# usra-riacs/Nonlocal-Monte-Carlo

Hardware: AMD Instinct MI355X
Metric: spin-updates/s (replicas x spins x sweeps / s), NPT sweep + swap rounds, schedule construction included (higher is better)
Workload: dtype f64 field + 53-bit uniform (the reference's arithmetic, NMC/nmc.py:86-87; on this +-J instance the fp64 field is an exact integer and the fp64 acceptance test an exact integer threshold per field value: bit-identical to the sweep-by-sweep fp64 kernel and the fp64 oracle); 1 GPU; NPT heat-bath sweeps + replica exchange, sparse +-J spin glass (C4 per GPU); spins=10000, edges=30000, replicas_per_gpu=256, replicas_total=256, sweeps_per_round=10, swap_pairs_per_round=77, rng=philox4x32-10, order=one permutation per sweep, plan_chunk_rounds=256

## Files before the change

nonlocal-monte-carlo_amd/csrc/nlmc.hip:

```cpp
#include "../../include/nlmc.h"
#include "nlmc_kernels.h"
#include "nlmc_pt_icm.h"
#include "nlmc_apt.h"
#include "nlmc_lbp.h"
#include "nlmc_nmc.h"
#include "nlmc_probe.h"
#include "nlmc_big.h"
#include "nlmc_host.h"

#include <dlfcn.h>

#include <algorithm>
#include <chrono>
#include <thread>
#include <climits>
#include <cmath>
#include <cstdio>
#include <cstdlib>
#include <cstring>
#include <string>
#include <vector>

namespace {

// ... 256 lines not shown
{
    const size_t i = 3 * t;
    const uint8_t kind = t < c->ev_kind.size() ? c->ev_kind[t] : 0;
    lev = sw = 0.f;
    HIP_TRY(c, hipEventSynchronize(c->events[i + 2]));
    if (kind == 0) {
        HIP_TRY(c, hipEventElapsedTime(&lev, c->events[i], c->events[i + 1]));
        HIP_TRY(c, hipEventElapsedTime(&sw, c->events[i + 1], c->events[i + 2]));
    } else if (kind == 1) {
        HIP_TRY(c, hipEventElapsedTime(&sw, c->events[i], c->events[i + 2]));
    } else {
        HIP_TRY(c, hipEventElapsedTime(&lev, c->events[i], c->events[i + 2]));
    }
    return NLMC_OK;
}

int sweep_block(int n)
{
    if (const char *s = getenv("NLMC_SWEEP_NT")) {
        int v = atoi(s);
        if (v >= 64 && v <= 1024 && v % 64 == 0) return v;
    }
    int nt = ((n + 7) / 8 + 63) / 64 * 64;
    return std::min(1024, std::max(64, nt));
}

int sweep_block_for(int n, bool f64_philox, bool f32_diag = false)
{
    return std::min(f64_philox ? 512 : f32_diag ? 768 : 1024, sweep_block(n));
}

int ensure_lds(nlmc_ctx *c, int slot, const void *func, size_t bytes)
{
    if (bytes > (size_t)158 * 1024) return fail(c, NLMC_ERR_UNSUPPORTED, "instance too large for the LDS-resident kernels of this build");
    if (bytes <= (size_t)60 * 1024 || bytes <= c->lds_opt[slot]) return NLMC_OK;
    HIP_TRY(c, hipFuncSetAttribute(func, hipFuncAttributeMaxDynamicSharedMemorySize, (int)bytes));
    c->lds_opt[slot] = bytes;
    return NLMC_OK;
}

int level_block(int n)
{
    int nt = ((n + 3) / 4 + 63) / 64 * 64;
    return std::min(1024, std::max(64, nt));
}

void launch_energy(nlmc_ctx *c, unsigned count, hipStream_t st, const EnergyArgs &a)
{
    const dim3 nt(c->n >= 4096 ? 1024 : 256);
    if (c->big) hipLaunchKernelGGL(k_energy<true>, dim3(count), nt, 0, st, a);
    else hipLaunchKernelGGL(k_energy<false>, dim3(count), nt, (size_t)c->n_pad, st, a);
}

int launch_energy_self(nlmc_ctx *c, double *dev_out)
{
    EnergyArgs a{};
    a.g = c->g;
    a.spins = c->spins.p;
    a.stride = c->n_pad;
    a.out = dev_out;
    a.efix = c->efix.p;
    a.escale = c->escale;
    if (c->n_chains > 0) launch_energy(c, (unsigned)c->n_chains, c->stream, a);
    HIP_TRY(c, hipGetLastError());
    return NLMC_OK;
}

int run_levelize(nlmc_ctx *c, int n_orders, const uint32_t *keys_in, int per_chain, int n_sweeps, uint32_t sweep0,
                 uint64_t seed, nlmc_ctx::Sched &sc, int ell_mode)
{
    if (n_orders <= 0) return NLMC_OK;
    if (ell_mode < 0) {
        BigLevelizeArgs b{};
        b.g = c->g;
        b.n_orders = n_orders;
        b.keys_in = keys_in;
        b.seed_lo = (uint32_t)seed; b.seed_hi = (uint32_t)(seed >> 32); b.sweep0 = sweep0;
        b.per_chain = per_chain; b.n_sweeps = n_sweeps; b.chain_base = c->chain_base;
        b.key = sc.bkey.p; b.lvl = sc.blvl.p; b.cur = sc.bcur.p;
        b.ord2 = sc.order.p; b.lvl_off = sc.lvl_off.p; b.nlev = sc.nlev.p; b.hi_max = sc.hi_max.p;
        HIP_TRY(c, c->big_flag.reserve(NLMC_BIG_PASSES));
        b.flag = c->big_flag.p;
        const unsigned gx = (unsigned)((c->n + 255) / 256);
        for (int ob = 0; ob < n_orders; ob += 65535) {
            const int no = std::min(65535, n_orders - ob);
            BigLevelizeArgs q = b;
            const size_t n = (size_t)c->n;
            q.n_orders = no;
            if (q.keys_in) q.keys_in += (size_t)ob * n;
            q.key = b.key ? b.key + (size_t)ob * n : nullptr; q.lvl += (size_t)ob * n; q.cur += (size_t)ob * (n + 2);
            q.ord2 += (size_t)ob * n; q.lvl_off += (size_t)ob * (n + 1); q.nlev += ob; q.hi_max += ob;
            if (!q.keys_in && per_chain && n_orders > 65535) return fail(c, NLMC_ERR_UNSUPPORTED, "more than 65535 per-chain orders of a long chain in one window");
            if (!q.keys_in) q.sweep0 = sweep0 + (uint32_t)ob;
            hipLaunchKernelGGL(k_blv_init, dim3(gx, no), dim3(256), 0, c->cur, q);
            HIP_TRY(c, hipGetLastError());
            bool settled = false;
            for (long long done = 0; !settled && done <= (long long)c->n + NLMC_BIG_PASSES; done += NLMC_BIG_PASSES) {
                int32_t fl[NLMC_BIG_PASSES];
                HIP_TRY(c, hipMemsetAsync(q.flag, 0, sizeof(fl), c->cur));
                for (int p = 0; p < NLMC_BIG_PASSES; ++p) hipLaunchKernelGGL(k_blv_pass, dim3(gx, no), dim3(256), 0, c->cur, q, p);
                HIP_TRY(c, hipGetLastError());
                HIP_TRY(c, hipMemcpyAsync(fl, q.flag, sizeof(fl), hipMemcpyDeviceToHost, c->cur));
                HIP_TRY(c, hipStreamSynchronize(c->cur));
                for (int p = 0; p < NLMC_BIG_PASSES; ++p) settled = settled || fl[p] == 0;
            }
            if (!settled) return fail(c, NLMC_ERR_STATE, "level schedule of a long chain did not settle");
            const unsigned gt = (unsigned)((c->n + NLMC_BIG_TILE - 1) / NLMC_BIG_TILE);
            hipLaunchKernelGGL(k_blv_hist, dim3(gt, no), dim3(256), 0, c->cur, q);
            hipLaunchKernelGGL(k_blv_scan, dim3(no), dim3(1024), 0, c->cur, q);
            hipLaunchKernelGGL(k_blv_place, dim3(gt, no), dim3(256), 0, c->cur, q);
            HIP_TRY(c, hipGetLastError());
        }
        return NLMC_OK;
    }
    LevelizeArgs a{};
    a.g = c->g;
    a.n_orders = n_orders;
    a.keys_in = keys_in;
    a.seed_lo = (uint32_t)seed;
    a.seed_hi = (uint32_t)(seed >> 32);
    a.sweep0 = sweep0;
    a.per_chain = per_chain;
    a.n_sweeps = n_sweeps;
    a.chain_base = c->chain_base;
    a.level_cap = sweep_block_for(c->n, ell_mode == 2, ell_mode == 1 && c->has_diag);
    a.ord2 = sc.order.p;
    a.lvl_off = sc.lvl_off.p;
    a.nlev = sc.nlev.p;
    a.hi_max = sc.hi_max.p;
    if (ell_mode == 1) { a.ell32 = sc.ell32.p; a.head32 = sc.head32.p; }
    if (ell_mode == 2) { a.ellc64 = sc.ellc64.p; a.ellv64 = sc.ellv64.p; a.headh64 = sc.headh64.p; a.pack16 = c->f64_pack16 ? 1 : 0; }
    const size_t lds_one = (size_t)(c->n + 2) * 4 + (((size_t)c->n * 2 + 3) / 4) * 4;
    const size_t lds_two = lds_one + (size_t)(c->n + 2) * 4;
    a.two_sided = lds_two + 16 <= (size_t)150 * 1024;
    const size_t lds = (a.two_sided ? lds_two : lds_one) + 16;
    { int rc = ensure_lds(c, 0, reinterpret_cast<const void *>(k_levelize), lds); if (rc) return rc; }
    hipLaunchKernelGGL(k_levelize, dim3(n_orders), dim3(level_block(c->n)), lds, c->cur, a);
    HIP_TRY(c, hipGetLastError());
    return NLMC_OK;
}

int fused_block(int n)
{
    if (getenv("NLMC_SWEEP_NT")) return std::max(256, sweep_block(n));
    const int nt = ((3 * n + 15) / 16 + 63) / 64 * 64;
    return std::min(1024, std::max(256, nt));
}

int fused_workers(int nt)
{
    const int waves = nt / 64;
    if (waves < 16) return waves - 1;
    if (const char *s = getenv("NLMC_FUSED_WORKERS")) { const int v = atoi(s); if (v >= 8 && v <= 16) return v; }
    return 15;
}

struct FusedLds { int neg_off, flags_off, u_off, u_bytes, snap_off, red_off, kt_off; size_t total; };
FusedLds fused_lds(int n, int n_pad, bool has_flags, bool with_out, bool with_neg, int kt_entries = 0)
{
    (void)n;
    FusedLds L{};
    L.neg_off = with_neg ? n_pad + 16 : 0;
    L.flags_off = (n_pad + 16) * (with_neg ? 2 : 1);
    int cur = L.flags_off + (has_flags ? n_pad + 16 : 0);
    cur = (cur + 15) / 16 * 16;
    L.u_off = cur;
    L.u_bytes = n_pad * 4;
    cur += 3 * L.u_bytes;
    L.snap_off = cur;
    if (with_out) cur += 3 * n_pad + 16;
    L.red_off = cur;
    L.kt_off = cur + 32;
    L.total = (size_t)cur + 32 + (size_t)kt_entries * 8;
    return L;
}

bool fused_addr_format(const nlmc_ctx *c)
{
    return c->sign8 && 2 * (c->n_pad + 16) <= 0xFFFF && fused_lds(c->n, c->n_pad, true, false, true).total <= (size_t)150 * 1024;
}

int fused_pstride(int n, int n_long, int T) { return (int)((((size_t)T * ((size_t)n + n_long) + 63) / 64 + NLMC_LCAP) * 64); }

int fused_gen0(int nt)
{
    const int waves = nt / 64;
    if (const char *s = getenv("NLMC_FUSED_GEN0")) { const int v = atoi(s); if (v >= 0 && v < waves) return v; }
    return waves / 2;
}

bool fused_supported(const nlmc_ctx *c, int T)
{
    if (getenv("NLMC_NO_FUSED") || c->big) return false;
    if (c->n < 256 || c->n > NLMC_FZ_SPT * 1024 || c->max_deg > 0x3FFF || T < 3 || T > NLMC_FUSED_TMAX) return false;
    if ((size_t)T * ((size_t)c->n + c->n_long) > ((size_t)1 << 22)) return false;
    if (c->n_pad + 16 > 0x3FFF) return false;
    (void)T;
    const FusedLds L = fused_lds(c->n, c->n_pad, true, false, false);
    if (3 * L.u_bytes / 4 > 0xFFFF) return false;
    return L.total <= (size_t)150 * 1024;
}

bool fused_f64_supported(const nlmc_ctx *c, int T)
{
    if (!c->f64_exact || c->xmax > 4095 || getenv("NLMC_NO_FUSED64")) return false;
    if (!fused_supported(c, T)) return false;
    return fused_lds(c->n, c->n_pad, false, false, fused_addr_format(c), 2 * c->xmax + 1).total <= (size_t)156 * 1024;
}

const void *fused_kernel(bool diag, bool flags, bool outs, int fmt, bool f64 = false)
{
    if (f64) {
#define NLMC_K64(D, O) {reinterpret_cast<const void *>(k_sweep_fused<D, false, O, NLMC_FMT_WIDE, true>), reinterpret_cast<const void *>(k_sweep_fused<D, false, O, NLMC_FMT_COMPACT, true>), \
                        reinterpret_cast<const void *>(k_sweep_fused<D, false, O, NLMC_FMT_ADDR, true>)}
        static const void *const t64[2][2][3] = {{NLMC_K64(false, false), NLMC_K64(false, true)}, {NLMC_K64(true, false), NLMC_K64(true, true)}};
#undef NLMC_K64
        return flags ? nullptr : t64[diag][outs][fmt];
    }
#define NLMC_K(D, F, O) {reinterpret_cast<const void *>(k_sweep_fused<D, F, O, NLMC_FMT_WIDE>), reinterpret_cast<const void *>(k_sweep_fused<D, F, O, NLMC_FMT_COMPACT>), \
                         reinterpret_cast<const void *>(k_sweep_fused<D, F, O, NLMC_FMT_ADDR>)}
    static const void *const table[2][2][2][3] = {{{NLMC_K(false, false, false), NLMC_K(false, false, true)}, {NLMC_K(false, true, false), NLMC_K(false, true, true)}},
                                                  {{NLMC_K(true, false, false), NLMC_K(true, false, true)}, {NLMC_K(true, true, false), NLMC_K(true, true, true)}}};
#undef NLMC_K
    static_assert(NLMC_FMT_WIDE == 0 && NLMC_FMT_COMPACT == 1 && NLMC_FMT_ADDR == 2, "table order");
    return table[diag][flags][outs][fmt];
}

struct SweepOut {
    int record_stride;
    int8_t *out_spins;
    double *out_energy;
    double *out_min_energy;
    int32_t *out_argmin;
    int8_t *out_argmin_state;
};

int run_fused(nlmc_ctx *c, int slot, int w, uint32_t sweep0, uint64_t seed, const double *tab_dev, int tab_cs, int tab_ss, bool use_slots,
              bool outs, bool want_energy, bool want_min, bool want_state, int rec, int t0, int n_total, bool f64 = false,
              const DeferSwap *defer = nullptr, double *sink_override = nullptr)
{
    const nlmc_ctx::FusedPlan &P = c->fz[slot];
    const int R = c->sub_count(), n = c->n, T = P.T;
    const size_t PS = (size_t)P.pstride;
    const int kt = f64 ? 2 * c->xmax + 1 : 0;
    const bool snap_lds = outs && fused_lds(c->n, c->n_pad, c->has_flags, true, P.fmt == NLMC_FMT_ADDR, kt).total <= (size_t)150 * 1024;
    const FusedLds L = fused_lds(c->n, c->n_pad, c->has_flags, snap_lds, P.fmt == NLMC_FMT_ADDR, kt);
    if (outs && !snap_lds) HIP_TRY(c, c->snap_g.reserve((size_t)R * (3 * (size_t)c->n_pad + 16)));
    const int variant = (outs ? 4 : 0) + (c->has_diag ? 2 : 0) + (c->has_flags ? 1 : 0);
    const void *kfun = fused_kernel(c->has_diag, c->has_flags, outs, P.fmt, f64);
    int lds_slot = f64 ? 48 + ((c->has_diag ? 2 : 0) + (outs ? 1 : 0)) * 3 + P.fmt : 24 + variant * 3 + P.fmt;
    if (defer) {
#define NLMC_KD(D, F64_) {reinterpret_cast<const void *>(k_sweep_fused<D, false, false, NLMC_FMT_WIDE, F64_, true>), reinterpret_cast<const void *>(k_sweep_fused<D, false, false, NLMC_FMT_COMPACT, F64_, true>), \
                          reinterpret_cast<const void *>(k_sweep_fused<D, false, false, NLMC_FMT_ADDR, F64_, true>)}
        static const void *const dtable[2][2][3] = {{NLMC_KD(false, false), NLMC_KD(false, true)}, {NLMC_KD(true, false), NLMC_KD(true, true)}};
#undef NLMC_KD
        kfun = (c->has_flags || outs) ? nullptr : dtable[c->has_diag][f64][P.fmt];
        lds_slot = 72 + ((c->has_diag ? 2 : 0) + (f64 ? 1 : 0)) * 3 + P.fmt;
    }
    if (!kfun) return fail(c, NLMC_ERR_STATE, "run_fused: no kernel for this combination (fp64 mode or deferred swap with phase flags / outputs)");
    { int rc = ensure_lds(c, lds_slot, kfun, L.total); if (rc) return rc; }
    const bool timed = c->ev_accumulate && (c->ev_every <= 1 || c->launches_total % c->ev_every == 0);
    hipEvent_t e0 = nullptr, e2 = nullptr;
    if (timed) {
        e0 = next_event(c);
        hipEvent_t e1 = next_event(c);
        e2 = next_event(c);
        if (!e0 || !e1 || !e2) return fail(c, NLMC_ERR_HIP, "hipEventCreate failed");
        tag_triple(c, 1);
        HIP_TRY(c, hipEventRecord(e0, c->cur));
    }
    SweepArgs a{};
    a.g = c->g;
    a.chain_base = c->chain_base;
    a.chain_list = c->sub_list();
    a.spins = c->spins.p;
    a.flags = c->has_flags ? c->flags.p : nullptr;
    a.temp_x = c->temp_x;
    a.lvl_off = P.loff.p + (size_t)w * (NLMC_LCAP + 1);
    a.nlev = P.nlev.p + w;
    a.hi_max = P.himax.p + w;
    a.ell32 = P.ell.p + (size_t)w * PS * NLMC_FZ_W;
    a.head32 = P.head.p + (size_t)w * PS;
    a.fsend = P.send.p + (size_t)w * T;
    a.fz_pstride = P.pstride;
    a.fz_fmt = P.fmt;
    if (w + 1 < P.windows && P.nlev_host[(size_t)w + 1] > 0 && !c->knob_no_warm) {
        a.warm_head = P.head.p + (size_t)(w + 1) * PS;
        a.warm_ell = P.ell.p + (size_t)(w + 1) * PS * NLMC_FZ_W;
        a.fz_npos_next = P.npos_host[(size_t)w + 1];
    }
    a.f_workers = P.workers;
    a.f_gen0 = P.gen0;
    a.f_gen_prio = c->knob_no_prio ? 0 : 1;
#ifdef NLMC_DEBUG_KNOBS
    a.dbg_flags = c->knob_dbg_flags;
#endif
    a.n_sweeps = T;
    a.sweep0 = sweep0;
    a.seed_lo = (uint32_t)seed; a.seed_hi = (uint32_t)(seed >> 32);
    a.tab = tab_dev; a.tab_cs = tab_cs; a.tab_ss = tab_ss;
    a.slot_of_chain = use_slots ? c->slot_of_chain.p : nullptr;
    a.efix = c->efix.p;
    a.energy_sink = sink_override ? sink_override : c->energy_sink;
    if (defer) a.defer = *defer;
    a.escale = c->escale;
    a.eshift = c->escale - c->qs;
    a.qinv = std::ldexp(1.0f, -c->qs);
// ... 2431 lines not shown
```

nonlocal-monte-carlo_amd/csrc/nlmc_kernels.h:

```cpp
#pragma once
#include "nlmc_device.h"

struct EdgeQ { int32_t col; int32_t q; };

struct CsrDev {
    int n, n_pad;
    const int32_t *rowptr;
    const int32_t *col;
    const double *val64;
    const EdgeQ *edge32;
    const double *h64;
    const int32_t *hq;
};

struct LevelizeArgs {
    CsrDev g;
    int n_orders;
    const uint32_t *keys_in;
    uint32_t seed_lo, seed_hi, sweep0;
    int per_chain;
    int n_sweeps;
    int chain_base;
    int level_cap;
    int two_sided;
// ... 1294 lines not shown
                const int l = l0 + (tid & 63);
                const unsigned long long m = __ballot((l < nl) && (loff[l + 1] - loff[l] > 64));
                if (m) n_bar = l0 + 64 - __clzll((long long)m);
            }
            const bool role_long = (Pf<T, PK>::W > 8) && ((tid & ~63) < a.hi_max[oid]);
            if (role_long) run_levels<T, DIAG, true, false, NoGen, PK>(a, x, ur, loff, so, nl, n_bar, cb0, cb1, esc);
            else run_levels<T, DIAG, false, false, NoGen, PK>(a, x, ur, loff, so, nl, n_bar, cb0, cb1, esc);

            if (dbuf && t + 1 < a.n_sweeps) {
                const int oid_n = a.per_chain ? (x.ob * a.n_sweeps + t + 1) : (t + 1);
                const int nl_n = a.nlev[oid_n];
                const bool wave0_busy = n_bar < nl;
                if (nl_n < NLMC_LCAP && (!wave0_busy || nt > 64)) {
                    const int hid = wave0_busy ? tid - 64 : tid, hcnt = wave0_busy ? nt - 64 : nt;
                    if (hid >= 0) {
                        T *ur_n = reinterpret_cast<T *>(reinterpret_cast<unsigned char *>(ur0) + (size_t)(pb ^ 1) * a.lds_u_stride);
                        int *loff_n = reinterpret_cast<int *>(reinterpret_cast<unsigned char *>(loff0) + (size_t)(pb ^ 1) * a.lds_loff_stride);
                        const int32_t *__restrict__ off_n = a.lvl_off + (size_t)oid_n * (n + 1);
                        fill_uniforms(ur_n, n, tt + 1u, gc, a.seed_lo, a.seed_hi, hid, hcnt);
                        for (int l = hid; l <= nl_n; l += hcnt) loff_n[l] = off_n[l];
                    }
                    prefilled = true;
                }
            }
        } else {
            for (int l = 0; l < nl; ++l) {
                const int lo = off[l], hi = off[l + 1];
                for (int i = lo + tid; i < hi; i += nt) {
                    Pf<T, PK> pe;
                    typename Pf<T, PK>::View vw;
                    vw.bind(a, so, n);
                    pe.template issue<true>(vw, i, true);
                    update_spin<T, DIAG, true, false, PK>(a, x, ur, pe, so, i, cb0, cb1, esc);
                }
                __syncthreads();
            }
        }
#ifdef NLMC_STAMPS
        const long long e0 = (long long)__builtin_readcyclecounter();
#endif
        __syncthreads();
        sweep_epilogue(a, x, t);
#ifdef NLMC_STAMPS
        st_epi += (long long)__builtin_readcyclecounter() - e0;
#endif
    }
#ifdef NLMC_STAMPS
    if (a.dbg && (tid & 63) == 0) {
        long long *d = a.dbg + ((size_t)c * 16 + (tid >> 6)) * 8;
        d[0] = st_u[0]; d[1] = st_u[1]; d[2] = st_u[2]; d[3] = st_u[3]; d[4] = st_u[4]; d[5] = st_fill;
        d[6] = (long long)__builtin_readcyclecounter() - st_begin; d[7] = st_epi;
    }
#endif
    chain_store(a, x);
}

template <int FMT> struct FusedItem {
    static constexpr int NE = NLMC_FZ_W;
    static constexpr int NP = FMT == NLMC_FMT_WIDE ? NE / 2 : FMT == NLMC_FMT_COMPACT ? NE / 4 : NE / 8;
    nlmc_i2 hd;
    nlmc_i4 pk[NP];
    __device__ __forceinline__ int word(int i) const { const int p = i >> 2, j = i & 3; return j == 0 ? pk[p].x : j == 1 ? pk[p].y : j == 2 ? pk[p].z : pk[p].w; }
    __device__ __forceinline__ unsigned col(int q) const
    {
        if (FMT == NLMC_FMT_WIDE) return (unsigned)word(2 * q);
        if (FMT == NLMC_FMT_COMPACT) return (unsigned)word(q) >> 16;
        return (q & 1) ? (unsigned)word(q >> 1) >> 16 : (unsigned)word(q >> 1) & 0xFFFFu;
    }
    __device__ __forceinline__ int val(int q) const
    {
        if (FMT == NLMC_FMT_WIDE) return word(2 * q + 1);
        return (int)(short)(word(q) & 0xFFFF);
    }
};

__device__ __forceinline__ float4 thresholds4(const u32x4 &r)
{
    float4 v;
    v.x = threshold_spec(r.x);
    v.y = threshold_spec(r.y);
    v.z = threshold_spec(r.z);
    v.w = threshold_spec(r.w);
    return v;
}

struct FusedGenParams { uint32_t gc; int gtid, gnt, nblk, nj, Tn; };
struct FusedWin {
    const int32_t *lvl_off;
    const int32_t *fsend;
    const EdgeQ *ell;
    const int2 *head;
    const int2 *warm_head;
    const EdgeQ *warm_ell;
    int npos_next;
    int nl, hi_max;
    uint32_t sweep0;
};
#ifdef NLMC_DEBUG_KNOBS
#define NLMC_GEN_DBG_OFF_COND (a.dbg_flags & 1)
#define NLMC_GEN_DBG_PHILOX if (a.dbg_flags & 8) g_r = u32x4{(uint32_t)b * 2654435761u, (uint32_t)b ^ gp.gc, (uint32_t)g_u * 40503u + (uint32_t)b, ~(uint32_t)b}; else
#define NLMC_GEN_DBG_LOGIT if (a.dbg_flags & 16) dst[b] = nlmc_f4{__uint_as_float(g_r.x & 0x3FFFFFFFu), __uint_as_float(g_r.y & 0x3FFFFFFFu), __uint_as_float(g_r.z & 0x3FFFFFFFu), __uint_as_float(g_r.w & 0x3FFFFFFFu)}; else
#else
#define NLMC_GEN_DBG_OFF_COND false
#define NLMC_GEN_DBG_PHILOX
#define NLMC_GEN_DBG_LOGIT
#endif
#define NLMC_GEN_STATE int g_u = 2, g_slot = 2, g_w0 = 0, g_wend = 0, g_wlen = 1, g_acc = 0, g_sidx = 0; u32x4 g_r{0u, 0u, 0u, 0u}; \
    const uint32_t g_seed_lo = a.seed_lo, g_seed_hi = a.seed_hi, g_sweep0 = W.sweep0; const int g_u_off = a.lds_u_off, g_u_stride = a.lds_u_stride; \
    const int32_t *const g_fsend = W.fsend;
#define NLMC_GEN_NSTEP (g_f64 ? 2 : 3)
#define NLMC_GEN_ARM(a, gp)                                                                                             \
    {                                                                                                                   \
        typedef const int32_t __attribute__((address_space(4))) *const_i32_;                                            \
        g_sidx = 0; g_acc = 0;                                                                                          \
        if (g_u < gp.Tn) {                                                                                              \
            const const_i32_ send_ = (const_i32_)(uintptr_t)g_fsend;                                                    \
            g_w0 = g_u >= 3 ? __builtin_amdgcn_readfirstlane(send_[g_u - 3]) : -1;                                      \
            g_wend = __builtin_amdgcn_readfirstlane(send_[g_u - 2]);                                                    \
            g_wlen = max(1, g_wend - g_w0);                 \
        } else g_w0 = 0x7FFFFFFF;                                                                                       \
    }
#define NLMC_GEN_STEP(a, gp)                                                                                            \
    {                                                                                                                   \
        const int call_ = g_sidx / NLMC_GEN_NSTEP, ph_ = g_sidx - call_ * NLMC_GEN_NSTEP;                               \
        const int b = gp.gtid + call_ * gp.gnt;                                                                         \
        if (ph_ == 0) {                                                                                                 \
            NLMC_GEN_DBG_PHILOX                                                                                         \
            g_r = philox4x32_rounds(u32x4{(uint32_t)b, g_sweep0 + (uint32_t)g_u, gp.gc, NLMC_TAG_UNIFORM}, g_seed_lo, g_seed_hi, 0, 5); \
        } else if (g_f64) {                                                                                             \
            typedef nlmc_i4 __attribute__((address_space(3))) *lds_i4_;                                                 \
            g_r = philox4x32_rounds(g_r, g_seed_lo, g_seed_hi, 5, 5);                                                   \
            if (b < gp.nblk) ((lds_i4_)(uintptr_t)(unsigned)(g_u_off + g_slot * g_u_stride))[b] = nlmc_i4{(int)(g_r.x >> 5), (int)(g_r.y >> 5), (int)(g_r.z >> 5), (int)(g_r.w >> 5)}; \
        } else if (ph_ == 1) {                                                                                          \
            NLMC_GEN_DBG_PHILOX                                                                                         \
            g_r = philox4x32_rounds(g_r, g_seed_lo, g_seed_hi, 5, 5);                                                   \
        } else if (b < gp.nblk) {                                                                                       \
            typedef nlmc_f4 __attribute__((address_space(3))) *lds_f4_;             \
            const lds_f4_ dst = (lds_f4_)(uintptr_t)(unsigned)(g_u_off + g_slot * g_u_stride);                  \
            NLMC_GEN_DBG_LOGIT                                                                                          \
            { const float4 t4 = thresholds4(g_r); dst[b] = nlmc_f4{t4.x, t4.y, t4.z, t4.w}; }                           \
        }                                                                                                               \
        ++g_sidx;                                                                                                       \
    }
#define NLMC_GEN(a, gp, l)                                                                                              \
    if (!(NLMC_GEN_DBG_OFF_COND) && (l) > g_w0) {                                                                       \
        g_acc += NLMC_GEN_NSTEP * gp.nj;                                                                                \
        while (g_acc >= g_wlen) { g_acc -= g_wlen; if (g_sidx < NLMC_GEN_NSTEP * gp.nj) NLMC_GEN_STEP(a, gp) }          \
        if (__builtin_expect((l) == g_wend, 0)) {                                                                       \
            while (g_sidx < NLMC_GEN_NSTEP * gp.nj) NLMC_GEN_STEP(a, gp)                                                \
            ++g_u; g_slot = g_slot == 2 ? 0 : g_slot + 1; NLMC_GEN_ARM(a, gp)                                           \
        }                                                                                                               \
    }

template <bool DIAG, bool FLAGS, bool PAIR, bool GEN, int FMT, bool OUT = false, bool F64 = false>
__device__ __forceinline__ void fused_levels(const SweepArgs &a, const FusedWin &W, unsigned char *lds_raw, int wv, int lane, int nl, float cq0,
                                             float cq1, long long &e_loc, const FusedGenParams gp)
{
    constexpr bool g_f64 = F64;
    static_assert(!(F64 && FLAGS), "fused fp64 windows: plain chains only (a scaled row's field is not an exact integer)");
    NLMC_GEN_STATE
    NLMC_GEN_ARM(a, gp)
    typedef const int32_t __attribute__((address_space(4))) *const_i32o;
    typedef const double __attribute__((address_space(4))) *const_f64o;
    const int o_npad = a.g.n_pad, o_b = blockIdx.x, o_c = a.chain_list ? a.chain_list[o_b] : o_b, o_tid = wv * 64 + lane;
    int o_t = 0, o_end = 0;
    unsigned o_lo = 0u;
    long long e_new = 0, E_run = 0, E_min = 0;
    int a_min = 0;
    float cqo0 = cq0, cqo1 = cq1, cqn0 = cq0, cqn1 = cq1;
    const int o_row = a.slot_of_chain ? a.slot_of_chain[a.chain_base + o_c] : o_c;
    int8_t *const snapg = (OUT && a.snap_g) ? a.snap_g + (size_t)o_b * (3 * (size_t)o_npad + 16) : nullptr;
#define NLMC_OCQ(t, j) ((float)((const_f64o)(uintptr_t)a.tab)[(size_t)o_row * a.tab_cs + (size_t)min((t), a.n_sweeps - 1) * a.tab_ss + (j)] * a.qinv)
    if (OUT) {
        o_end = ((const_i32o)(uintptr_t)W.fsend)[0];
        E_run = uniform64(a.efix[o_c]);
        E_min = a.emin ? uniform64(a.emin[o_c]) : 0x7FFFFFFFFFFFFFFFll;
        a_min = a.emin ? __builtin_amdgcn_readfirstlane(a.argmin[o_c]) : 0;
        cqn0 = NLMC_OCQ(1, 0); cqn1 = NLMC_OCQ(1, 1);
    }
    typedef FusedItem<FMT> Item;
    unsigned v_u_off = (unsigned)a.lds_u_off, v_neg_off = (unsigned)a.lds_neg_off;
    int v_eshift = a.eshift;
    asm volatile("" : "+v"(v_u_off), "+v"(v_neg_off), "+v"(v_eshift));
    unsigned v_kt0 = (unsigned)(a.lds_kt_off + 4 * a.f64_xmax), v_tie = a.f64_tie_mask;
    if (F64) asm volatile("" : "+v"(v_kt0), "+v"(v_tie));
    typedef const unsigned __attribute__((address_space(3))) *lds_u32;
    constexpr int NP = Item::NP, NE = Item::NE;
    const int plane_bytes = a.fz_pstride * 16;
    const __amdgpu_buffer_rsrc_t r_ell = __builtin_amdgcn_make_buffer_rsrc(const_cast<EdgeQ *>(W.ell), 0, (NLMC_FZ_W / 2) * plane_bytes, 0x00020000);
    const __amdgpu_buffer_rsrc_t r_head = __builtin_amdgcn_make_buffer_rsrc(const_cast<int2 *>(W.head), 0, a.fz_pstride * 8, 0x00020000);
    typedef const int32_t __attribute__((address_space(4))) *const_i32;
    const const_i32 loffp = (const_i32)(uintptr_t)W.lvl_off;
    auto lo = [&](int i) __attribute__((always_inline)) { return loffp[min(i, nl)]; };
    const int lane16 = lane * 16, oob = 0x7FF00000;
    typedef const int8_t __attribute__((address_space(3))) *lds_i8;
    typedef int8_t __attribute__((address_space(3))) *lds_i8w;
    typedef const uint8_t __attribute__((address_space(3))) *lds_u8;
    typedef const float __attribute__((address_space(3))) *lds_f32;

    auto issue = [&](Item &it, int c, bool has) __attribute__((always_inline)) {
#ifdef NLMC_DEBUG_KNOBS
        if (a.dbg_flags & 32) return;
#endif
        const int v16 = has ? lane16 : oob;
        it.hd = __builtin_amdgcn_raw_buffer_load_b64(r_head, v16 >> 1, c * 512, 0);
#pragma unroll
        for (int q = 0; q < NP; ++q) it.pk[q] = __builtin_amdgcn_raw_buffer_load_b128(r_ell, v16, c * 1024 + q * plane_bytes, 0);
    };
    auto update = [&](const Item &it, int lv) __attribute__((always_inline)) {
        (void)lv;
#ifdef NLMC_DEBUG_KNOBS
        if (a.dbg_flags & 2) { asm volatile("" :: "v"(it.hd.x), "v"(it.pk[0].x), "v"(it.pk[Item::NP - 1].x)); return; }
#endif
        const int hx = it.hd.x;
#ifdef NLMC_DEBUG_KNOBS
        const unsigned ka = (a.dbg_flags & 1024) ? (unsigned)((lane & 31) * 4 + (lane >> 5)) : (unsigned)hx & 0x3FFFu;
        const float wk = *(lds_f32)(uintptr_t)(((a.dbg_flags & 1024) ? (unsigned)(lane * 4) : (((unsigned)hx >> 16) << 2)) + (unsigned)a.lds_u_off);
#else
        const unsigned ka = (unsigned)hx & 0x3FFFu;
        const float wk = *(lds_f32)(uintptr_t)((((unsigned)hx >> 16) << 2) + v_u_off);
#endif
        int so = (int)*(lds_i8)(uintptr_t)ka;
        unsigned f = 0u;
        if (FLAGS) f = (unsigned)*(lds_u8)(uintptr_t)(ka + (unsigned)a.lds_flags_off);
        int sj[NE];
#ifdef NLMC_DEBUG_KNOBS
        if (a.dbg_flags & 512) {
#pragma unroll
            for (int q = 0; q < NE; ++q) sj[q] = (int)*(lds_i8)(uintptr_t)(unsigned)((lane & 31) * 4 + q * 132 + (lane >> 5));
        } else
#endif
        {
#pragma unroll
            for (int q = 0; q < NE; ++q) sj[q] = (int)*(lds_i8)(uintptr_t)it.col(q);
        }
        asm volatile("" : "+v"(so));
        int X0 = it.hd.y, X1 = 0, Xd = 0;
#pragma unroll
        for (int q = 0; q < NE; q += 2) {
            if (FMT == NLMC_FMT_ADDR) {
                X0 += sj[q];
                X1 += sj[q + 1];
            } else {
                X0 += __mul24(it.val(q), sj[q]);
                X1 += __mul24(it.val(q + 1), sj[q + 1]);
            }
        }
        if (DIAG) {
#pragma unroll
            for (int q = 0; q < NE; ++q) {
                if (FMT == NLMC_FMT_ADDR) Xd += (it.col(q) == ka || it.col(q) == ka + v_neg_off) ? sj[q] : 0;
                else Xd += (it.col(q) == ka) ? __mul24(it.val(q), sj[q]) : 0;
            }
        }
        int X = X0 + X1;
        bool second = false;
        if (PAIR) {
            if (__builtin_amdgcn_ballot_w64((hx & 0x4000) != 0) != 0ull) {
                if (hx & 0x4000) {
                    const int rs = a.g.rowptr[ka], re = a.g.rowptr[ka + 1];
#pragma clang loop vectorize(disable) unroll(disable)
                    for (int e = rs + 2 * NLMC_FZ_W; e < re; ++e) {
                        const EdgeQ t = a.g.edge32[e];
                        const int pr = __mul24(t.q, (int)*(lds_i8)(uintptr_t)(unsigned)t.col);
                        X += pr;
                        if (DIAG && (unsigned)t.col == ka) Xd += pr;
                    }
                }
            }
            const bool pair = (hx & 0x8000) != 0;
            const int Xp = __builtin_amdgcn_mov_dpp(X, 0xB1, 0xF, 0xF, true);
            X += pair ? Xp : 0;
            if (DIAG) { const int Xdp = __builtin_amdgcn_mov_dpp(Xd, 0xB1, 0xF, 0xF, true); Xd += pair ? Xdp : 0; }
            second = pair && (lane & 1);
        }
        bool up64 = false;
        if (F64) {
            const unsigned hk = __float_as_uint(wk);
            const unsigned kaddr = ((unsigned)X << 2) + v_kt0;
#ifdef NLMC_DEBUG_KNOBS
            const unsigned kh = (a.dbg_flags & 16384) ? (unsigned)(X * 3000000 + 0x4000000) : *(lds_u32)(uintptr_t)kaddr;
#else
            const unsigned kh = *(lds_u32)(uintptr_t)kaddr;
#endif
            up64 = hk < kh;
            const bool tie = ((hk ^ kh) & v_tie) == 0u;
            if (__builtin_expect(__builtin_amdgcn_ballot_w64(tie) != 0ull, 0)) {
                if (tie) {
                    typedef const int32_t __attribute__((address_space(4))) *const_i32s;
                    const unsigned tw_ = (unsigned)hx >> 16, np_ = (unsigned)a.g.n_pad;
                    int t_ = tw_ >= 3u * np_ ? 3 : tw_ >= 2u * np_ ? 2 : tw_ >= np_ ? 1 : 0;
                    while (t_ + 3 < a.n_sweeps && lv > ((const_i32s)(uintptr_t)W.fsend)[t_]) t_ += 3;
                    const u32x4 r_ = philox4x32_10(ka >> 2, W.sweep0 + (uint32_t)t_, gp.gc, NLMC_TAG_UNIFORM_LO, a.seed_lo, a.seed_hi);
                    const unsigned lw_ = (ka & 2u) ? ((ka & 1u) ? r_.w : r_.z) : ((ka & 1u) ? r_.y : r_.x);
                    const unsigned lo_ = lw_ >> 6;
                    const unsigned kl = *(lds_u32)(uintptr_t)(kaddr + 4u * (unsigned)(2 * a.f64_xmax + 1));
                    up64 = hk < kh || (hk == kh && lo_ < kl);
                }
            }
        }
        if (!OUT) {
            const float z = ((FLAGS && f == 1u) ? cq1 : cq0) * (float)X;
            int sn = F64 ? (up64 ? 1 : -1) : (z < wk) ? 1 : -1;
            if (FLAGS) sn = (f >= 2u) ? so : sn;
            const int cv = (PAIR && second) ? 0 : (so - sn) << v_eshift;
            e_loc += (long long)(DIAG ? X - Xd : X) * (long long)cv;
            *(lds_i8w)(uintptr_t)ka = (int8_t)sn;
            if (FMT == NLMC_FMT_ADDR) *(lds_i8w)(uintptr_t)(ka + v_neg_off) = (int8_t)-sn;
        } else {
            const unsigned tw = (unsigned)hx >> 16;
            const bool is_old = tw - o_lo < (unsigned)o_npad;
            const float cqa = is_old ? cqo0 : cqn0, cqb = is_old ? cqo1 : cqn1;
            const float z = ((FLAGS && f == 1u) ? cqb : cqa) * (float)X;
            int sn = F64 ? (up64 ? 1 : -1) : (z < wk) ? 1 : -1;
            if (FLAGS) sn = (f >= 2u) ? so : sn;
            const int cv = (PAIR && second) ? 0 : (so - sn) << v_eshift, cvo = is_old ? cv : 0;
            const long long Xt = (long long)(DIAG ? X - Xd : X);
            e_loc += Xt * (long long)cvo;
            e_new += Xt * (long long)(cv - cvo);
            *(lds_i8w)(uintptr_t)ka = (int8_t)sn;
            if (FMT == NLMC_FMT_ADDR) *(lds_i8w)(uintptr_t)(ka + v_neg_off) = (int8_t)-sn;
            if (snapg) snapg[tw] = (int8_t)sn;
            else *(lds_i8w)(uintptr_t)(tw + (unsigned)a.lds_snap_off) = (int8_t)sn;
        }
    };
#define NLMC_OUT_PRE                                                                                                    \
    {                                                                                                                   \
        if (snapg) asm volatile("s_waitcnt vmcnt(0)" ::: "memory");            \
        const long long w_ = wave_sum_i64(e_loc);                                                                       \
        long long *red_ = reinterpret_cast<long long *>(lds_raw + a.lds_red_off);                                       \
        if (lane == 0 && w_ != 0) atomicAdd(reinterpret_cast<unsigned long long *>(&red_[o_t % 3]), (unsigned long long)w_); \
    }
#define NLMC_OUT_POST                                                                                                   \
    {                                                                                                                   \
        long long *red_ = reinterpret_cast<long long *>(lds_raw + a.lds_red_off);                                       \
        const int slot_ = o_t % 3, tg_ = a.t0 + o_t;                                                                    \
        E_run += uniform64(red_[slot_]);                                                                                \
        const bool better_ = a.emin && E_run < E_min && (tg_ % a.min_stride == 0);    \
        if (better_) { E_min = E_run; a_min = tg_; }                                                                    \
        if (o_tid == 0) {                                                                                               \
            red_[(o_t + 2) % 3] = 0;                                \
            if (a.etrace) a.etrace[(size_t)o_b * a.trace_sweeps + tg_] = E_run;                                         \
        }                                                                                                               \
        const unsigned char *snap_ = snapg ? reinterpret_cast<const unsigned char *>(snapg) + (size_t)slot_ * o_npad              \
                                           : lds_raw + a.lds_snap_off + (size_t)slot_ * o_npad;                         \
        if (better_ && a.best) {                                                                                        \
            int4 *dst_ = reinterpret_cast<int4 *>(a.best + (size_t)o_c * o_npad);                                       \
            const int4 *src_ = reinterpret_cast<const int4 *>(snap_);                                                   \
            if (snapg) for (int i_ = o_tid; i_ < o_npad / 16; i_ += a.f_workers * 64)                                  \
                reinterpret_cast<nlmc_i4 *>(dst_)[i_] = __builtin_nontemporal_load(&reinterpret_cast<const nlmc_i4 *>(src_)[i_]);   \
            else for (int i_ = o_tid; i_ < o_npad / 16; i_ += a.f_workers * 64) dst_[i_] = src_[i_];                    \
        }                                                                                                               \
        if (a.strace && tg_ % a.rec_stride == 0) {                                 \
            const int n_rec_ = (a.trace_sweeps + a.rec_stride - 1) / a.rec_stride;                                      \
            int8_t *dst_ = a.strace + ((size_t)o_b * n_rec_ + (size_t)(tg_ / a.rec_stride)) * a.g.n;                   \
            if (snapg) for (int i_ = o_tid; i_ < a.g.n; i_ += a.f_workers * 64) dst_[i_] = (int8_t)__builtin_nontemporal_load(&snap_[i_]); \
            else for (int i_ = o_tid; i_ < a.g.n; i_ += a.f_workers * 64) dst_[i_] = (int8_t)snap_[i_];                 \
        }                                                                                                               \
        e_loc = e_new; e_new = 0;                                                                                       \
        ++o_t;                                                                                                          \
        o_lo = (unsigned)((o_t % 3) * o_npad);                                                                          \
        o_end = o_t < a.n_sweeps ? ((const_i32o)(uintptr_t)W.fsend)[o_t] : 0x7FFFFFFF;                                   \
        cqo0 = cqn0; cqo1 = cqn1;                                                                                       \
        cqn0 = NLMC_OCQ(o_t + 1, 0); cqn1 = NLMC_OCQ(o_t + 1, 1);                                                       \
    }

#ifdef NLMC_STAMPS
    long long sw0, sw1, sw2, st_work = 0, st_bar = 0, st_calls = 0;
#endif
    {
        Item I0, I1, I2;
        int r0 = lo(0), r1 = lo(1), r2 = lo(2), r3 = lo(3), r4 = lo(4), r5 = lo(5);
        bool h0 = r0 + wv < r1, h1 = (1 < nl) && (r1 + wv < r2), h2;
        issue(I0, r0 + wv, h0);
        issue(I1, r1 + wv, h1);
#define NLMC_FSTAGE(lv, cur, hcur, nxt, hnxt, b2, b3)                                       \
        {                                                                                   \
            NLMC_FW0                                                                        \
            hnxt = ((lv) + 2 < nl) && ((b2) + wv < (b3));                                   \
            if (GEN) NLMC_GEN(a, gp, lv)                                                    \
            if (hcur) { update(cur, lv); NLMC_FCALL }                                       \
            issue(nxt, (b2) + wv, hnxt NLMC_DBG_NOLOAD);                                    \
            const bool end_ = OUT && __builtin_expect((lv) == o_end, 0);    \
            if (end_) NLMC_OUT_PRE                                                          \
            NLMC_FW1                                                                        \
            NLMC_DBG_BARRIER                                                                \
            NLMC_FW2                                                                        \
            if (end_) NLMC_OUT_POST                                                         \
        }
        for (int l = 0; l < nl; l += 3) {
            const int n3 = lo(l + 6), n4 = lo(l + 7), n5 = lo(l + 8);
            NLMC_FSTAGE(l, I0, h0, I2, h2, r2, r3)
            if (l + 1 < nl) NLMC_FSTAGE(l + 1, I1, h1, I0, h0, r3, r4)
            if (l + 2 < nl) NLMC_FSTAGE(l + 2, I2, h2, I1, h1, r4, r5)
            r0 = r3; r1 = r4; r2 = r5; r3 = n3; r4 = n4; r5 = n5;
        }
#undef NLMC_FSTAGE
    }
#ifdef NLMC_STAMPS
    if (a.dbg && lane == 0) {
        long long *d = a.dbg + ((size_t)blockIdx.x * 16 + wv) * 8;
        d[4] = st_calls; d[5] = st_work; d[6] = st_bar;
    }
#endif
    if (OUT && o_tid == 0) {
        a.efix[o_c] = E_run;
        if (a.energy_sink) a.energy_sink[o_c] = (double)E_run * __longlong_as_double((long long)(1023 - a.escale) << 52);
        if (a.emin) { a.emin[o_c] = E_min; a.argmin[o_c] = a_min; }
    }
}

template <bool FLAGS>
__device__ __forceinline__ void fused_state_load(const SweepArgs &a, unsigned char *lds_raw, int c)
{
    const int n_pad = a.g.n_pad, tid = threadIdx.x, nt = blockDim.x;
    long long *red = reinterpret_cast<long long *>(lds_raw + a.lds_red_off);
    {
        const int4 *src = reinterpret_cast<const int4 *>(a.spins + (size_t)c * n_pad);
        int4 *dst = reinterpret_cast<int4 *>(lds_raw);
        for (int i = tid; i < n_pad / 16; i += nt) dst[i] = src[i];
        if (tid < 4) reinterpret_cast<int *>(lds_raw + n_pad)[tid] = tid < 2 ? 0x01010101 : 0;
        if (a.lds_neg_off) {
            int4 *ndst = reinterpret_cast<int4 *>(lds_raw + a.lds_neg_off);
            for (int i = tid; i < n_pad / 16; i += nt) {
                const int4 v = src[i];
                ndst[i] = make_int4(v.x ^ (int)0xFEFEFEFE, v.y ^ (int)0xFEFEFEFE, v.z ^ (int)0xFEFEFEFE, v.w ^ (int)0xFEFEFEFE);
            }
            if (tid < 4) reinterpret_cast<int *>(lds_raw + a.lds_neg_off + n_pad)[tid] = (int)0xFFFFFFFF;
        }
        if (FLAGS) {
            const int4 *fsrc = reinterpret_cast<const int4 *>(a.flags + (size_t)c * n_pad);
            int4 *fdst = reinterpret_cast<int4 *>(lds_raw + a.lds_flags_off);
            for (int i = tid; i < n_pad / 16; i += nt) fdst[i] = fsrc[i];
            if (tid < 4) reinterpret_cast<int *>(lds_raw + a.lds_flags_off + n_pad)[tid] = 0;
        }
        if (tid < 4) red[tid] = 0;
    }
}

template <bool DIAG, bool FLAGS, bool OUT, int FMT, bool F64>
__device__ __forceinline__ void fused_window(const SweepArgs &a, const FusedWin &W, unsigned char *lds_raw, int row, uint32_t gc, long long &e_loc)
{
    constexpr bool g_f64 = F64;
    const int n = a.g.n, tid = threadIdx.x, nt = blockDim.x;
    const int wv = __builtin_amdgcn_readfirstlane(tid >> 6), lane = tid & 63;
    float *ur = reinterpret_cast<float *>(lds_raw + a.lds_u_off);
    const int Tn = a.n_sweeps;
#ifdef NLMC_DEBUG_KNOBS
    const int nl = (a.dbg_flags & 128) ? 0 : W.nl;
#else
    const int nl = W.nl;
#endif
    const float cq0 = (float)a.tab[(size_t)row * a.tab_cs] * a.qinv, cq1 = (float)a.tab[(size_t)row * a.tab_cs + 1] * a.qinv;
#ifdef NLMC_DEBUG_KNOBS
    for (int t = 0; t < ((a.dbg_flags & 1) ? 3 : min(2, Tn)) NLMC_DBG_NOPROLOGUE; ++t) {
#else
    for (int t = 0; t < min(2, Tn) NLMC_DBG_NOPROLOGUE; ++t) {
#endif
        float *tab_t = reinterpret_cast<float *>(reinterpret_cast<unsigned char *>(ur) + (size_t)t * a.lds_u_stride);
        if (F64) fill_uniform_words(reinterpret_cast<unsigned *>(tab_t), n, W.sweep0 + (uint32_t)t, gc, a.seed_lo, a.seed_hi, tid, nt);
        else fill_uniforms(tab_t, n, W.sweep0 + (uint32_t)t, gc, a.seed_lo, a.seed_hi, tid, nt);
    }
    if (F64) {
        const int ne = 2 * a.f64_xmax + 1;
        unsigned *kt = reinterpret_cast<unsigned *>(lds_raw + a.lds_kt_off);
        const double cb = a.tab[(size_t)row * a.tab_cs];
        for (int i = nt - 1 - tid; i < ne; i += nt) {
            const double xf = (double)(i - a.f64_xmax) * a.qinv64;
            const unsigned long long K = accept_count_spec(cb * xf);
            kt[i] = (unsigned)(K >> 26);
            kt[ne + i] = (unsigned)(K & 0x3FFFFFFull);
        }
    }
    __syncthreads();

    const int g0 = a.f_gen0 * 64, nblk = (n + 3) / 4, gnt = nt - g0;
    const int gwave0 = __builtin_amdgcn_readfirstlane((tid - g0) & ~63);
    const FusedGenParams gp{gc, tid - g0, gnt, nblk, max(0, (nblk - gwave0 + gnt - 1) / gnt), Tn};
    const bool is_gen = tid >= g0;
    if (is_gen && a.f_gen_prio) __builtin_amdgcn_s_setprio(2);
    if (wv < a.f_workers) {
        const bool role_long = wv < W.hi_max;
        const int variant = (role_long ? 2 : 0) + (is_gen ? 1 : 0);
#define NLMC_FL(P, G) fused_levels<DIAG, FLAGS, P, G, FMT, OUT, F64>(a, W, lds_raw, wv, lane, nl, cq0, cq1, e_loc, gp)
        switch (variant) { case 0: NLMC_FL(false, false); break; case 1: NLMC_FL(false, true); break;
                           case 2: NLMC_FL(true, false); break; default: NLMC_FL(true, true); break; }
#undef NLMC_FL
    } else {
        NLMC_GEN_STATE
        NLMC_GEN_ARM(a, gp)
        const int hid = tid - a.f_workers * 64, hcnt = nt - a.f_workers * 64;
        const unsigned warm_lines = W.warm_head ? (unsigned)(((size_t)W.npos_next * 8 + 127) / 128) : 0u;
        const unsigned warm_lines_p = W.warm_head ? (unsigned)(((size_t)a.fz_pstride * 16 + 127) / 128) : 0u;
        const unsigned warm_used_p = W.warm_head ? (unsigned)(((size_t)W.npos_next * 16 + 127) / 128) : 0u;
        const unsigned warm_total = warm_lines + (FMT == NLMC_FMT_ADDR ? 1u : FMT == NLMC_FMT_COMPACT ? 2u : 4u) * warm_used_p;
        unsigned warm_at = (unsigned)blockIdx.x * (unsigned)hcnt + (unsigned)hid;
        const unsigned warm_step = gridDim.x * (unsigned)hcnt;
        unsigned wv0 = 0u, wv1 = 0u, wv2 = 0u, wv3 = 0u;
        auto warm_addr = [&]() __attribute__((always_inline)) -> const unsigned * {
            const char *p = reinterpret_cast<const char *>(W.lvl_off);
            if (warm_at < warm_lines) p = reinterpret_cast<const char *>(W.warm_head) + (size_t)warm_at * 128;
            else if (warm_at < warm_total) {
                const unsigned r = warm_at - warm_lines, q = r / warm_used_p, i = r - q * warm_used_p;
                p = reinterpret_cast<const char *>(W.warm_ell) + ((size_t)q * warm_lines_p + i) * 128;
            }
            warm_at = warm_at < warm_total ? warm_at + warm_step : warm_at;
            return reinterpret_cast<const unsigned *>(p);
        };
#define NLMC_WARM(reg) { asm volatile("" :: "v"(reg) : "memory"); reg = *warm_addr(); }
#ifdef NLMC_STAMPS
        long long sw0, sw1, sw2, st_work = 0, st_bar = 0;
#endif
        for (int l = 0; l < nl; l += 4) {
            NLMC_FW0
            NLMC_WARM(wv0)
            if (is_gen) NLMC_GEN(a, gp, l)
            NLMC_FW1
            __syncthreads();
            NLMC_FW2
            if (l + 1 < nl) { NLMC_FW0 NLMC_WARM(wv1) if (is_gen) NLMC_GEN(a, gp, l + 1) NLMC_FW1 __syncthreads(); NLMC_FW2 }
            if (l + 2 < nl) { NLMC_FW0 NLMC_WARM(wv2) if (is_gen) NLMC_GEN(a, gp, l + 2) NLMC_FW1 __syncthreads(); NLMC_FW2 }
            if (l + 3 < nl) { NLMC_FW0 NLMC_WARM(wv3) if (is_gen) NLMC_GEN(a, gp, l + 3) NLMC_FW1 __syncthreads(); NLMC_FW2 }
        }
#ifdef NLMC_STAMPS
        if (a.dbg && lane == 0) {
            long long *d = a.dbg + ((size_t)blockIdx.x * 16 + wv) * 8;
            d[5] = st_work; d[6] = st_bar;
        }
#endif
        auto warm_next = [&]() __attribute__((always_inline)) { NLMC_WARM(wv0) };
        while (warm_at < warm_total) warm_next();
        asm volatile("" :: "v"(wv0), "v"(wv1), "v"(wv2), "v"(wv3) : "memory");
#undef NLMC_WARM
    }

}

template <bool OUT>
__device__ __forceinline__ void fused_state_store(const SweepArgs &a, unsigned char *lds_raw, int c, long long e_loc)
{
    const int n_pad = a.g.n_pad, tid = threadIdx.x, nt = blockDim.x, lane = tid & 63;
    long long *red = reinterpret_cast<long long *>(lds_raw + a.lds_red_off);
    {
        const long long w = OUT ? 0ll : wave_sum_i64(e_loc);
        if (lane == 0 && w != 0) atomicAdd(reinterpret_cast<unsigned long long *>(&red[3]), (unsigned long long)w);
        __syncthreads();
        int4 *dst = reinterpret_cast<int4 *>(a.spins + (size_t)c * n_pad);
        const int4 *src = reinterpret_cast<const int4 *>(lds_raw);
        for (int i = tid; i < n_pad / 16; i += nt) dst[i] = src[i];
        if (tid == 0 && !OUT) {
            const long long E = a.efix[c] + red[3];
            a.efix[c] = E;
            if (a.energy_sink) a.energy_sink[c] = (double)E * __longlong_as_double((long long)(1023 - a.escale) << 52);
        }
    }
}

template <bool ATOMIC>
__device__ __forceinline__ int pt_swap_step_of_chain(int slot, uint32_t gc, int lane, int L, int n_pairs, int n_ladders, uint32_t round,
                                                     const int32_t *sel_round, const double *beta, int32_t *slot_of_chain, int32_t *chain_of_slot,
                                                     double Ed, const double *e_all, int32_t *log_pairs, uint8_t *log_acc, uint32_t seed_lo,
                                                     uint32_t seed_hi)
{
    (void)n_ladders;
    const int g = (int)gc / L;
    const int32_t *sel = sel_round + (size_t)g * n_pairs * 2;
    int fp = -1, fi = 0, out = slot;
    for (int p0 = 0; p0 < n_pairs; p0 += 64) {
        const int p = p0 + lane;
        const int i = p < n_pairs ? sel[2 * p] : -5;
        const unsigned long long m = __ballot(i == slot || i + 1 == slot);
        if (m) { const int src = __ffsll((long long)m) - 1; fp = p0 + src; fi = __shfl(i, src, 64); break; }
    }
    if (fp >= 0) {
        const int i = fi, ps = slot == i ? i + 1 : i;
        int partner;
        double Ep;
        if (ATOMIC) {
            partner = __hip_atomic_load(&chain_of_slot[(size_t)g * L + ps], __ATOMIC_RELAXED, __HIP_MEMORY_SCOPE_AGENT);
            Ep = __hip_atomic_load(&e_all[partner], __ATOMIC_RELAXED, __HIP_MEMORY_SCOPE_AGENT);
        } else {
            partner = chain_of_slot[(size_t)g * L + ps];
            Ep = e_all[partner];
        }
        const double Ea = slot == i ? Ed : Ep, Eb = slot == i ? Ep : Ed;
        const double dE = Eb - Ea, dB = beta[i + 1] - beta[i];
        const u32x4 rr = philox4x32_10((uint32_t)fp, round, (uint32_t)g, NLMC_TAG_SWAP, seed_lo, seed_hi);
        const double u = uniform_from(rr, 0.0);
        const double z = (dB * dE) * 1.4426950408889634;
        const bool acc = u < exp2_spec(z);
        if (lane == 0) {
            if (slot == i && log_pairs) {
                const size_t at = (size_t)g * n_pairs + fp;
                log_pairs[2 * at] = i; log_pairs[2 * at + 1] = i + 1;
                log_acc[at] = acc ? 1 : 0;
            }
            if (acc) {
                if (ATOMIC) {
                    __hip_atomic_store(&slot_of_chain[gc], ps, __ATOMIC_RELAXED, __HIP_MEMORY_SCOPE_AGENT);
                    __hip_atomic_store(&chain_of_slot[(size_t)g * L + ps], (int)gc, __ATOMIC_RELAXED, __HIP_MEMORY_SCOPE_AGENT);
                } else {
                    slot_of_chain[gc] = ps;
                    chain_of_slot[(size_t)g * L + ps] = (int)gc;
                }
            }
        }
        if (acc) out = ps;
    }
    return out;
}

template <bool DIAG, bool FLAGS, bool OUT, int FMT, bool F64 = false, bool DEFER = false>
__global__ __launch_bounds__(1024) void k_sweep_fused(SweepArgs a)
{
    extern __shared__ __align__(16) unsigned char lds_raw[];
    if ((unsigned)reinterpret_cast<size_t>(lds_raw) != 0u) __builtin_trap();
    static_assert(!(DEFER && OUT), "the deferred swap rides on the plain variant");
    const int c = a.chain_list ? a.chain_list[blockIdx.x] : (int)blockIdx.x;
    const uint32_t gc_chain = (uint32_t)(a.chain_base + c);
    int row = a.slot_of_chain ? a.slot_of_chain[gc_chain] : c;
    int new_row = row;
    if (DEFER && a.defer.n_pairs > 0 && threadIdx.x < 64)
        new_row = pt_swap_step_of_chain<false>(row, gc_chain, (int)threadIdx.x, a.defer.ladder_len, a.defer.n_pairs, a.defer.n_ladders, a.defer.round,
                                               a.defer.plan_pairs, a.defer.beta, a.defer.slot_of_chain, a.defer.chain_of_slot,
                                               a.defer.e_prev[gc_chain], a.defer.e_prev, a.defer.log_pairs, a.defer.log_acc, a.seed_lo, a.seed_hi);
#ifdef NLMC_STAMPS
    const long long st_begin = (long long)__builtin_readcyclecounter();
#endif
    const FusedWin W{a.lvl_off, a.fsend, a.ell32, a.head32, a.warm_head, a.warm_ell, a.fz_npos_next, a.nlev[0], a.hi_max[0], a.sweep0};
    fused_state_load<FLAGS>(a, lds_raw, c);
    if (DEFER) {
        volatile int *sh = reinterpret_cast<volatile int *>(lds_raw + a.lds_red_off);
        __syncthreads();
        if (threadIdx.x == 0) sh[0] = new_row;
        __syncthreads();
        row = sh[0];
        __syncthreads();
        if (threadIdx.x == 0) sh[0] = 0;
    }
    const uint32_t gc = (a.rng_stride && a.slot_of_chain) ? (uint32_t)((c / a.rng_ladder_len) * a.rng_stride + a.rng_base + row) : gc_chain;
    long long e_loc = 0;
    fused_window<DIAG, FLAGS, OUT, FMT, F64>(a, W, lds_raw, row, gc, e_loc);
    fused_state_store<OUT>(a, lds_raw, c, e_loc);
#ifdef NLMC_STAMPS
    if (a.dbg && (threadIdx.x & 63) == 0) a.dbg[((size_t)blockIdx.x * 16 + (threadIdx.x >> 6)) * 8 + 7] = (long long)__builtin_readcyclecounter() - st_begin;
#endif
}

struct RoundsArgs {
    int n_rounds, n_windows_avail;
    const int32_t *loff, *nlev, *himax, *send, *npos;
    const int2 *head;
    const EdgeQ *ell;
    int ladder_len, n_pairs, n_ladders;
    uint32_t round0;
    const int32_t *plan_pairs;
    const double *beta;
    int32_t *slot_of_chain, *chain_of_slot;
    double *ebuf;
    int32_t *log_pairs;
    uint8_t *log_acc;
    unsigned *bar;
    int32_t *status;
    long long timeout_ticks;
};

__device__ __forceinline__ bool grid_arrive_and_wait(unsigned *bar, unsigned target, int32_t *status, long long t_end, volatile int *flag)
{
    if (threadIdx.x == 0) {
        asm volatile("s_waitcnt vmcnt(0)" ::: "memory");
        __hip_atomic_fetch_add(bar, 1u, __ATOMIC_RELAXED, __HIP_MEMORY_SCOPE_AGENT);
        int good = 1;
        while (__hip_atomic_load(bar, __ATOMIC_RELAXED, __HIP_MEMORY_SCOPE_AGENT) < target) {
            if (__hip_atomic_load(status, __ATOMIC_RELAXED, __HIP_MEMORY_SCOPE_AGENT) == 3 || (long long)wall_clock64() > t_end) {
                __hip_atomic_store(status, 3, __ATOMIC_RELAXED, __HIP_MEMORY_SCOPE_AGENT);
                good = 0;
                break;
            }
            __builtin_amdgcn_s_sleep(2);
        }
        *flag = good;
    }
    __syncthreads();
    return *flag != 0;
}

// ... 159 lines not shown
```

Measured before the change: 224.2 billion spin-updates/s.

## Use all 16 waves as workers, folding cache warming into last worker wave

The default fused worker count goes from 15 to 16 waves, so with a 1024-thread block no dedicated helper wave is left. To keep the L2 prefetch ('warm') of the next window's schedule data, the last generator worker wave now issues one warm load per level stage inside its sweep loop, then drains any remaining warm loads at the end. This adds a sixteenth wave of spin-update work per block, at the cost of extra loads and register pressure on one worker wave. It may also unbalance the per-level work across waves.

```diff
diff --git a/nonlocal-monte-carlo_amd/csrc/nlmc.hip b/nonlocal-monte-carlo_amd/csrc/nlmc.hip
--- a/nonlocal-monte-carlo_amd/csrc/nlmc.hip
+++ b/nonlocal-monte-carlo_amd/csrc/nlmc.hip
@@ -432,7 +432,7 @@
     const int waves = nt / 64;
     if (waves < 16) return waves - 1;
     if (const char *s = getenv("NLMC_FUSED_WORKERS")) { const int v = atoi(s); if (v >= 8 && v <= 16) return v; }
-    return 15;
+    return 16;
 }
 
 struct FusedLds { int neg_off, flags_off, u_off, u_bytes, snap_off, red_off, kt_off; size_t total; };
diff --git a/nonlocal-monte-carlo_amd/csrc/nlmc_kernels.h b/nonlocal-monte-carlo_amd/csrc/nlmc_kernels.h
--- a/nonlocal-monte-carlo_amd/csrc/nlmc_kernels.h
+++ b/nonlocal-monte-carlo_amd/csrc/nlmc_kernels.h
@@ -1470,7 +1470,26 @@
         }                                                                                                               \
     }
 
-template <bool DIAG, bool FLAGS, bool PAIR, bool GEN, int FMT, bool OUT = false, bool F64 = false>
+#define NLMC_WARM_STATE(hid_, hcnt_)                                                                                    \
+    const unsigned warm_lines = W.warm_head ? (unsigned)(((size_t)W.npos_next * 8 + 127) / 128) : 0u;            \
+    const unsigned warm_lines_p = W.warm_head ? (unsigned)(((size_t)a.fz_pstride * 16 + 127) / 128) : 0u;   \
+    const unsigned warm_used_p = W.warm_head ? (unsigned)(((size_t)W.npos_next * 16 + 127) / 128) : 0u;       \
+    const unsigned warm_total = warm_lines + (FMT == NLMC_FMT_ADDR ? 1u : FMT == NLMC_FMT_COMPACT ? 2u : 4u) * warm_used_p; \
+    unsigned warm_at = (unsigned)blockIdx.x * (unsigned)(hcnt_) + (unsigned)(hid_);                                      \
+    const unsigned warm_step = gridDim.x * (unsigned)(hcnt_);                                                            \
+    auto warm_addr = [&]() __attribute__((always_inline)) -> const unsigned * {                                          \
+        const char *p = reinterpret_cast<const char *>(W.lvl_off);                                                       \
+        if (warm_at < warm_lines) p = reinterpret_cast<const char *>(W.warm_head) + (size_t)warm_at * 128;               \
+        else if (warm_at < warm_total) {                                                                                 \
+            const unsigned r = warm_at - warm_lines, q = r / warm_used_p, i = r - q * warm_used_p;                        \
+            p = reinterpret_cast<const char *>(W.warm_ell) + ((size_t)q * warm_lines_p + i) * 128;                       \
+        }                                                                                                                \
+        warm_at = warm_at < warm_total ? warm_at + warm_step : warm_at;                                                  \
+        return reinterpret_cast<const unsigned *>(p);                                                                    \
+    };
+#define NLMC_WARM(reg) { asm volatile("" :: "v"(reg) : "memory"); reg = *warm_addr(); }
+
+template <bool DIAG, bool FLAGS, bool PAIR, bool GEN, int FMT, bool OUT = false, bool F64 = false, bool WARM = false>
 __device__ __forceinline__ void fused_levels(const SweepArgs &a, const FusedWin &W, unsigned char *lds_raw, int wv, int lane, int nl, float cq0,
                                              float cq1, long long &e_loc, const FusedGenParams gp)
 {
@@ -1688,13 +1707,16 @@
 #endif
     {
         Item I0, I1, I2;
+        unsigned wr0 = 0u, wr1 = 0u, wr2 = 0u;
+        NLMC_WARM_STATE(lane, 64)
         int r0 = lo(0), r1 = lo(1), r2 = lo(2), r3 = lo(3), r4 = lo(4), r5 = lo(5);
         bool h0 = r0 + wv < r1, h1 = (1 < nl) && (r1 + wv < r2), h2;
         issue(I0, r0 + wv, h0);
         issue(I1, r1 + wv, h1);
-#define NLMC_FSTAGE(lv, cur, hcur, nxt, hnxt, b2, b3)                                       \
+#define NLMC_FSTAGE(lv, cur, hcur, nxt, hnxt, b2, b3, wr)                                   \
         {                                                                                   \
             NLMC_FW0                                                                        \
+            if (WARM) NLMC_WARM(wr)                                                         \
             hnxt = ((lv) + 2 < nl) && ((b2) + wv < (b3));                                   \
             if (GEN) NLMC_GEN(a, gp, lv)                                                    \
             if (hcur) { update(cur, lv); NLMC_FCALL }                                       \
@@ -1708,12 +1730,16 @@
         }
         for (int l = 0; l < nl; l += 3) {
             const int n3 = lo(l + 6), n4 = lo(l + 7), n5 = lo(l + 8);
-            NLMC_FSTAGE(l, I0, h0, I2, h2, r2, r3)
-            if (l + 1 < nl) NLMC_FSTAGE(l + 1, I1, h1, I0, h0, r3, r4)
-            if (l + 2 < nl) NLMC_FSTAGE(l + 2, I2, h2, I1, h1, r4, r5)
+            NLMC_FSTAGE(l, I0, h0, I2, h2, r2, r3, wr0)
+            if (l + 1 < nl) NLMC_FSTAGE(l + 1, I1, h1, I0, h0, r3, r4, wr1)
+            if (l + 2 < nl) NLMC_FSTAGE(l + 2, I2, h2, I1, h1, r4, r5, wr2)
             r0 = r3; r1 = r4; r2 = r5; r3 = n3; r4 = n4; r5 = n5;
         }
 #undef NLMC_FSTAGE
+        if (WARM) {
+            while (warm_at < warm_total) NLMC_WARM(wr0)
+            asm volatile("" :: "v"(wr0), "v"(wr1), "v"(wr2) : "memory");
+        }
     }
 #ifdef NLMC_STAMPS
     if (a.dbg && lane == 0) {
@@ -1800,32 +1826,18 @@
     if (wv < a.f_workers) {
         const bool role_long = wv < W.hi_max;
         const int variant = (role_long ? 2 : 0) + (is_gen ? 1 : 0);
-#define NLMC_FL(P, G) fused_levels<DIAG, FLAGS, P, G, FMT, OUT, F64>(a, W, lds_raw, wv, lane, nl, cq0, cq1, e_loc, gp)
-        switch (variant) { case 0: NLMC_FL(false, false); break; case 1: NLMC_FL(false, true); break;
-                           case 2: NLMC_FL(true, false); break; default: NLMC_FL(true, true); break; }
+        const bool warm = a.f_workers * 64 == nt && wv == a.f_workers - 1 && is_gen;
+#define NLMC_FL(P, G, WM) fused_levels<DIAG, FLAGS, P, G, FMT, OUT, F64, WM>(a, W, lds_raw, wv, lane, nl, cq0, cq1, e_loc, gp)
+        if (warm) { if (role_long) NLMC_FL(true, true, true); else NLMC_FL(false, true, true); }
+        else switch (variant) { case 0: NLMC_FL(false, false, false); break; case 1: NLMC_FL(false, true, false); break;
+                                case 2: NLMC_FL(true, false, false); break; default: NLMC_FL(true, true, false); break; }
 #undef NLMC_FL
     } else {
         NLMC_GEN_STATE
         NLMC_GEN_ARM(a, gp)
         const int hid = tid - a.f_workers * 64, hcnt = nt - a.f_workers * 64;
-        const unsigned warm_lines = W.warm_head ? (unsigned)(((size_t)W.npos_next * 8 + 127) / 128) : 0u;
-        const unsigned warm_lines_p = W.warm_head ? (unsigned)(((size_t)a.fz_pstride * 16 + 127) / 128) : 0u;
-        const unsigned warm_used_p = W.warm_head ? (unsigned)(((size_t)W.npos_next * 16 + 127) / 128) : 0u;
-        const unsigned warm_total = warm_lines + (FMT == NLMC_FMT_ADDR ? 1u : FMT == NLMC_FMT_COMPACT ? 2u : 4u) * warm_used_p;
-        unsigned warm_at = (unsigned)blockIdx.x * (unsigned)hcnt + (unsigned)hid;
-        const unsigned warm_step = gridDim.x * (unsigned)hcnt;
+        NLMC_WARM_STATE(hid, hcnt)
         unsigned wv0 = 0u, wv1 = 0u, wv2 = 0u, wv3 = 0u;
-        auto warm_addr = [&]() __attribute__((always_inline)) -> const unsigned * {
-            const char *p = reinterpret_cast<const char *>(W.lvl_off);
-            if (warm_at < warm_lines) p = reinterpret_cast<const char *>(W.warm_head) + (size_t)warm_at * 128;
-            else if (warm_at < warm_total) {
-                const unsigned r = warm_at - warm_lines, q = r / warm_used_p, i = r - q * warm_used_p;
-                p = reinterpret_cast<const char *>(W.warm_ell) + ((size_t)q * warm_lines_p + i) * 128;
-            }
-            warm_at = warm_at < warm_total ? warm_at + warm_step : warm_at;
-            return reinterpret_cast<const unsigned *>(p);
-        };
-#define NLMC_WARM(reg) { asm volatile("" :: "v"(reg) : "memory"); reg = *warm_addr(); }
 #ifdef NLMC_STAMPS
         long long sw0, sw1, sw2, st_work = 0, st_bar = 0;
 #endif
@@ -1849,7 +1861,6 @@
         auto warm_next = [&]() __attribute__((always_inline)) { NLMC_WARM(wv0) };
         while (warm_at < warm_total) warm_next();
         asm volatile("" :: "v"(wv0), "v"(wv1), "v"(wv2), "v"(wv3) : "memory");
-#undef NLMC_WARM
     }
 
 }
```

Measured after the change: 226.9 billion spin-updates/s, median of 6. 1.2% higher.
